# eth-cscs/COSTA

Measured on AMD Instinct MI355X. Metric: GB/s device-resident tile pack+transpose+unpack (fp64), % HBM peak, higher is better.
Workload: dtype f64; 1 GPU; pxtran fp64 16384x16384, 256x256 blocks, op T, alpha=1 beta=0, 1x1 grid (BASELINE configs[1]); op=T, parallelism=1 rank(s), one per GPU, RCCL send/recv exchange, m=16384, n=16384, block=256, grid=1x1

## Files before the change

costa_amd/__init__.py:

```python
from __future__ import annotations

import ctypes as C
import os
import struct
from dataclasses import dataclass
from typing import Iterable, Sequence

import numpy as np

__all__ = [
    "CostaError", "lib", "FLOAT", "DOUBLE", "CFLOAT", "CDOUBLE", "INT32", "dtype_code",
    "np_dtype", "Layout", "block_cyclic_layout", "custom_layout", "Comm", "transform",
    "transform_batch", "transform_async", "transform_batch_async", "synchronize", "transformer", "copy_and_transform", "execute_tiles", "execute_tiles_mixed",
    "convert_subtile", "TileOp",
    "plan_export", "set_profiling", "get_stats", "release_caches", "TILE_OP_DTYPE",
]

FLOAT, DOUBLE, CFLOAT, CDOUBLE, INT32 = 0, 1, 2, 3, 4
_NP = {FLOAT: np.float32, DOUBLE: np.float64, CFLOAT: np.complex64,
       CDOUBLE: np.complex128, INT32: np.int32}

TILE_TRANSPOSE, TILE_CONJ, TILE_VEC_SRC, TILE_VEC_DST = 0x1, 0x2, 0x4, 0x8
SCALE_BITCOPY, SCALE_ZERO, SCALE_ALPHA, SCALE_AXPBY = 0, 1, 2, 3

# ... 54 lines not shown
                ("plan_misses", C.c_int64), ("host_groups", C.c_int64),
                ("device_plans", C.c_int64), ("plan_ms", C.c_double), ("host_direct", C.c_int64),
                ("host_direct_groups", C.c_int64), ("tile_items", C.c_int64), ("skew_items", C.c_int64),
                ("cblock_items", C.c_int64), ("tiny_items", C.c_int64), ("device_lists", C.c_int64),
                ("fused_pieces", C.c_int64)]

    def as_dict(self) -> dict:
        out = {}
        for cls in reversed(type(self).__mro__):
            for k, _ in cls.__dict__.get("_fields_", ()):
                out[k] = getattr(self, k)
        return out


class FullStats(Stats):
    _fields_ = [("convert_items", C.c_int64)]


LIB_PATH = os.environ.get("COSTA_LIB") or os.path.join(os.path.dirname(os.path.abspath(__file__)),
                                                       "lib", "libcosta_amd.so")
_lib = None


def lib():
    global _lib
    if _lib is not None:
        return _lib
    if not os.environ.get("COSTA_NO_TORCH"):
        try:
            import torch
        except Exception:
# ... 2 lines not shown
        raise CostaError(-1, f"native library missing: {LIB_PATH} (run __graft_entry__.build())")
    L = C.CDLL(LIB_PATH, mode=C.RTLD_GLOBAL)
    vp, i, c, i64 = C.c_void_p, C.c_int, C.c_char, C.c_int64
    sig = {
        "costa_hip_last_error": (C.c_char_p, []),
        "costa_hip_version": (i, []),
        "costa_hip_block_cyclic_layout": (i, [i, i, i, i, i, i, i, i, i, i, i, c, i, i, vp, i, c, i,
                                              C.POINTER(vp)]),
        "costa_hip_custom_layout": (i, [i, i, i, C.POINTER(i), C.POINTER(i), C.POINTER(i), i,
                                        C.POINTER(_Block), c, C.POINTER(vp)]),
        "costa_hip_layout_destroy": (None, [vp]),
        "costa_hip_layout_reorder_ranks": (i, [vp, C.POINTER(i), i]),
        "costa_hip_layout_num_blocks": (i, [vp]),
        "costa_hip_layout_block": (i, [vp, i, C.POINTER(i), C.POINTER(i), C.POINTER(i),
                                       C.POINTER(i), C.POINTER(vp), C.POINTER(i)]),
        "costa_hip_comm_self": (i, [i, C.POINTER(vp)]),
        "costa_hip_comm_unique_id": (i, [C.c_char_p]),
        "costa_hip_comm_create": (i, [C.c_char_p, i, i, i, C.POINTER(vp)]),
        "costa_hip_comm_rank": (i, [vp]),
        "costa_hip_comm_size": (i, [vp]),
        "costa_hip_comm_destroy": (None, [vp]),
        "costa_hip_transform": (i, [vp, vp, c, vp, vp, vp]),
        "costa_hip_transform_batch": (i, [i, C.POINTER(vp), C.POINTER(vp), C.c_char_p, vp, vp,
                                          vp]),
        "costa_hip_transform_async": (i, [vp, vp, c, vp, vp, vp, vp]),
        "costa_hip_transform_batch_async": (i, [i, C.POINTER(vp), C.POINTER(vp), C.c_char_p, vp,
                                                vp, vp, vp]),
        "costa_hip_synchronize": (i, [vp]),
        "costa_hip_device_count": (i, [C.POINTER(i)]),
        "costa_hip_rccl_version": (i, [C.POINTER(i)]),
# ... 71 lines not shown

    @property
    def handle(self) -> C.c_void_p:
        return self._h

    def num_blocks(self) -> int:
        return lib().costa_hip_layout_num_blocks(self._h)

    def block(self, i: int) -> BlockInfo:
        v = [C.c_int() for _ in range(4)]
        d, ld = C.c_void_p(), C.c_int()
        _check(lib().costa_hip_layout_block(self._h, i, *[C.byref(x) for x in v], C.byref(d),
                                            C.byref(ld)))
        return BlockInfo(v[0].value, v[1].value, v[2].value, v[3].value, d.value or 0, ld.value)

    def reorder_ranks(self, reordering: Sequence[int]):
        p = np.ascontiguousarray(reordering, dtype=np.int32)
        _check(lib().costa_hip_layout_reorder_ranks(self._h, p.ctypes.data_as(C.POINTER(C.c_int)),
                                                    int(p.size)))

    def close(self):
        if self._h and self._h.value:
            lib().costa_hip_layout_destroy(self._h)
            self._h = C.c_void_p(0)

    def __del__(self):
        try:
            self.close()
        except Exception:
            pass
# ... 299 lines not shown
```

costa_amd/csrc/capi.cpp:

```cpp
#include "engine.hpp"

#include <hip/hip_runtime.h>

#include <costa/transform.hpp>

#include <algorithm>
#include <cctype>
#include <complex>
#include <cstring>
#include <new>

struct costa_layout_s {
    costa::engine::elayout e;
    std::vector<int> base_owners;
};
struct costa_comm_s {
    costa::engine::comm* c = nullptr;
};

namespace {
thread_local std::string g_last_error;

template <typename F>
int guarded(F&& f) {
// ... 201 lines not shown
            if (seen[size_t(reordering[k])]++)
                throw costa::engine::error(COSTA_ERR_ARG, "costa: reordering is not a permutation");
        }
        std::vector<int> owners(base.size());
        for (size_t k = 0; k < base.size(); ++k) owners[k] = n > 0 ? reordering[base[k]] : base[k];
        e.owners = std::move(owners);
        e.n_ranks = std::max(e.n_ranks, n);
        costa::engine::set_layout_hash(e);
    });
}

int costa_hip_layout_num_blocks(costa_layout_t layout) {
    return layout ? int(layout->e.blocks.size()) : -1;
}

int costa_hip_layout_block(costa_layout_t layout, int i, int* row_start, int* row_end,
                           int* col_start, int* col_end, void** data, int* ld) {
    return guarded([&] {
        if (!layout || i < 0 || size_t(i) >= layout->e.blocks.size())
            throw costa::engine::error(COSTA_ERR_ARG, "block index out of range");
        const auto& b = layout->e.blocks[size_t(i)];
        if (row_start) *row_start = b.rows.start;
        if (row_end) *row_end = b.rows.end;
        if (col_start) *col_start = b.cols.start;
        if (col_end) *col_end = b.cols.end;
        if (data) *data = b.data;
        if (ld) *ld = b.ld;
    });
}

// ... 319 lines not shown
```

costa_amd/csrc/convert_kernels.hip:

```cpp
#include <hip/hip_runtime.h>

#include <algorithm>
#include <string>
#include <type_traits>

#include "engine.hpp"
#include "tile_device.hpp"

#pragma clang fp contract(off)

namespace costa {
namespace engine {
namespace {

template <typename Td, typename Ts>
struct conv_t {
    static __device__ __forceinline__ Td of(Ts x) { return static_cast<Td>(x); }
};
template <typename Rd, typename Rs>
struct conv_t<cpx<Rd>, cpx<Rs>> {
    static __device__ __forceinline__ cpx<Rd> of(cpx<Rs> x) {
        return {static_cast<Rd>(x.re), static_cast<Rd>(x.im)};
    }
};
// ... 107 lines not shown
template <typename Ts, typename Td, bool FULL>
__device__ __forceinline__ void run_convert(const costa_tile_op_t& op, int f0, int s0, int tf_, int ts_,
                                            const char* src_base, char* dst_base, Td alpha, Td beta,
                                            typename cshape<Ts, Td>::Tn* tile) {
    using S = cshape<Ts, Td>;
    using Tn = typename S::Tn;
    constexpr int V = S::V, P = S::P;
    const int tf = FULL ? S::BF : tf_;
    const int ts = FULL ? S::BS : ts_;
    const uint32_t flags = op.flags;
    const uint32_t kind = (flags & COSTA_SCALE_MASK) >> COSTA_SCALE_SHIFT;
    const bool conj = flags & COSTA_TILE_CONJ;
    const bool vs = FULL || (flags & COSTA_TILE_VEC_SRC);
    const bool vd = FULL || (flags & COSTA_TILE_VEC_DST);
    const int64_t lds = op.lds, ldd = op.ldd;
    const Ts* src = reinterpret_cast<const Ts*>(src_base + op.src) + int64_t(s0) * lds + f0;

    const int lf = (int(threadIdx.x) % S::LPC) * V;
    const int c0 = int(threadIdx.x) / S::LPC;
    auto col_of = [&](int k) { return c0 + k * S::CPP; };
    const int nf_lane = FULL ? V : tf - lf;
    strip<Ts, V> x[S::PL];
#pragma unroll
    for (int k = 0; k < S::PL; ++k) {
        const int s = col_of(k);
        if (FULL || (nf_lane > 0 && s < ts)) sload(x[k], src + s * lds + lf, nf_lane, vs);
    }

    if (!(flags & COSTA_TILE_TRANSPOSE)) {
        Td* dst = reinterpret_cast<Td*>(dst_base + op.dst) + int64_t(s0) * ldd + f0;
        strip<Td, V> y[S::PL];
        if (kind == COSTA_SCALE_AXPBY) {
#pragma unroll
            for (int k = 0; k < S::PL; ++k) {
                const int s = col_of(k);
                if (FULL || (nf_lane > 0 && s < ts)) sload(y[k], dst + s * ldd + lf, nf_lane, vd);
            }
        }
        uint32_t redo = 0;
#pragma unroll
        for (int k = 0; k < S::PL; ++k) {
            const int s = col_of(k);
            if (!FULL && (nf_lane <= 0 || s >= ts)) continue;
            strip<Td, V> o;
            bool bad = false;
// ... 15 lines not shown
                    if (!((redo >> k) & 1u)) continue;
                    const int s = col_of(k);
                    const Ts* a = src + s * lds + lf;
                    Td* d = dst + s * ldd + lf;
                    const int n = FULL ? V : min(V, nf_lane);
#pragma unroll 1
                    for (int e = 0; e < n; ++e)
                        d[e] = scale(conv<Td>(a[e]), kind == COSTA_SCALE_AXPBY ? d[e] : e_zero<Td>(),
                                     kind, conj, alpha, beta);
                }
            }
        }
        return;
    }

    Td* dst = reinterpret_cast<Td*>(dst_base + op.dst) + int64_t(f0) * ldd + s0;
    const int lane = int(threadIdx.x) % 64, wave = int(threadIdx.x) / 64;
    constexpr int SW = S::SW, QG = S::QG;
    auto unit = [&](int k, int& f, int& sb, int& n) {
        const int u = wave + S::NW * k;
        const int sc = u / QG, q = u % QG;
        const int j = lane & (V - 1);
        f = q * V + j;
        sb = sc * SW + (lane - j);
        n = FULL ? V : ts - sb;
        return FULL || (f < tf && n > 0);
    };
    strip<Td, V> old[S::PS];
    if (kind == COSTA_SCALE_AXPBY) {
#pragma unroll
        for (int k = 0; k < S::PS; ++k) {
// ... 193 lines not shown
```

costa_amd/csrc/engine.cpp:

```cpp
#include <exception>
#include <thread>
#include "engine.hpp"

#include <hip/hip_runtime.h>
#include <rccl/rccl.h>

#include <algorithm>
#include <numeric>
#include <chrono>
#include <cmath>
#include <cstdio>
#include <cstdlib>
#include <cstring>
#include <deque>
#include <list>
#include <map>
#include <mutex>
#include <unordered_map>

namespace costa {
namespace engine {

#define HIP_CHECK(x)                                                                   \
    do {                                                                               \
// ... 1389 lines not shown
        h2 = (h2 + v) * 0x9fb21c651e98df25ull;
        h2 ^= h2 >> 31;
    }
    void mix_vec(const std::vector<int>& v) {
        mix(v.size());
        for (int x : v) mix(uint64_t(uint32_t(x)));
    }
    void mix_layout(const elayout& L) {
        mix(uint64_t(L.dtype));
        mix(uint64_t(uint8_t(L.ordering)));
        mix(uint64_t(L.n_ranks));
        mix_vec(L.rows_split);
        mix_vec(L.cols_split);
        mix_vec(L.owners);
        mix(L.blocks.size());
        for (const auto& b : L.blocks) {
            mix(uint64_t(uint32_t(b.rows.start)) | (uint64_t(uint32_t(b.rows.end)) << 32));
            mix(uint64_t(uint32_t(b.cols.start)) | (uint64_t(uint32_t(b.cols.end)) << 32));
            mix(reinterpret_cast<uintptr_t>(b.data));
            mix(uint64_t(uint32_t(b.ld)));
        }
    }
};

}

uint64_t layout_hash(const elayout& L) {
    hasher h;
    h.mix_layout(L);
    return h.h | 1;
}

void layout_hashes(const elayout& L, uint64_t& h1, uint64_t& h2) {
    hasher h;
    h.mix_layout(L);
    h1 = h.h | 1;
    h2 = h.h2;
}

// ... 8 lines not shown
    std::vector<hrange> h2d_ranges, d2h_ranges;
    dbuf stage;
    dbuf d_local, w_local, d_scal;
    work_split l_local;
    bool tr_local = true, ax_local = true;
    convert_list c_local;
    struct xround {
        dbuf d_pack, w_pack, d_unpack, w_unpack;
        work_split l_pack, l_unpack;
        convert_list c_pack, c_unpack;
        bool tr_unpack = false, ax_unpack = false;
    };
    std::vector<std::unique_ptr<xround>> rounds;
    std::vector<unsigned char> scal_host;
    std::shared_ptr<host_pipeline> pipe;
};

constexpr size_t kMaxPlans = 16;
struct keyed_plan {
    uint64_t h = 0;
    std::vector<uint64_t> key;
    std::unique_ptr<cached_plan> plan;
};
std::list<keyed_plan> g_plans;

void key_layout(std::vector<uint64_t>& k, const elayout& L) {
    uint64_t h1 = L.hash, h2 = L.hash2;
    if (!h1) layout_hashes(L, h1, h2);
    k.push_back(h1);
    k.push_back(h2);
    k.push_back(uint64_t(L.dtype) | uint64_t(uint8_t(L.ordering)) << 8 |
                uint64_t(uint32_t(L.n_ranks)) << 32);
    k.push_back(uint64_t(uint32_t(L.nbr())) | uint64_t(uint32_t(L.nbc())) << 32);
    k.push_back(L.blocks.size());
    if (!L.blocks.empty())
        for (const eblock* b : {&L.blocks.front(), &L.blocks.back()}) {
            k.push_back(reinterpret_cast<uintptr_t>(b->data));
            k.push_back(uint64_t(uint32_t(b->ld)) | uint64_t(uint32_t(b->rows.start)) << 32);
        }
// ... 139 lines not shown
        key_layout(key, *j.C);
        uint64_t w = uint64_t(uint8_t(std::toupper(static_cast<unsigned char>(j.trans))));
        for (bool cm : {true, false})
            w = w << 8 | scale_kind(j.C->dtype, j.s, cm, std::toupper(j.trans) == 'C');
        key.push_back(w);
    }
    hasher h;
    for (uint64_t w : key) h.mix(w);
    for (auto it = g_plans.begin(); it != g_plans.end(); ++it) {
        if (it->h == h.h && it->key == key) {
            g_plans.splice(g_plans.begin(), g_plans, it);
            g_stats.plan_hits++;
            return g_plans.front().plan.get();
        }
    }
    g_stats.plan_misses++;
    static const bool trace = std::getenv("COSTA_PLAN_TRACE") != nullptr;
    auto now = [] {
        return std::chrono::duration<double, std::milli>(
                   std::chrono::steady_clock::now().time_since_epoch()).count();
    };
    const double t0 = now();
    double t_resid = 0, t_plan = 0, t_work = 0;

    const bool mixed = any_mixed(jobs);
    if (mixed) {
        costa_dtype_t a, b;
        check_jobs(jobs, c->size, a, b);
    }
    auto cp = std::make_unique<cached_plan>();
    cp->device = c->device;
    bool all_dev = true;
    std::vector<const elayout*> host_layouts;
    std::vector<bool> on_dev;
    for (const auto& j : jobs)
        for (const elayout* L : {j.A, j.C}) {
            bool d = layout_on_device(*L);
            on_dev.push_back(d);
            all_dev = all_dev && d;
        }
    std::vector<elayout> remapped;
    std::vector<job> pj = jobs;
    std::vector<hrange> staged_ranges;
    std::vector<uint8_t> range_flags;
    if (!all_dev && mixed)
        throw error(COSTA_ERR_ARG,
                    "costa: mixed-precision transforms (A and C of different element types) need "
                    "device-resident layouts");
    if (!all_dev) {
        cp->staged = true;
        std::vector<const elayout*> As, Cs;
        size_t k = 0;
        for (const auto& j : jobs) {
            if (!on_dev[k++]) As.push_back(j.A);
            if (!on_dev[k++]) Cs.push_back(j.C);
// ... 37 lines not shown
                       std::none_of(on_dev.begin(), on_dev.end(), [](bool d) { return d; });
        for (uint8_t f : range_flags)
            if ((f & 3) == 3 || (f & 4)) pipe_ok = false;
        if (pipe_ok) {
            const double tp = now();
            auto hplan = plan_jobs(jobs, c, dc.main);
            g_stats.plan_ms += now() - tp;
            if (host_pipeline_accepts(hplan->dtype, hplan->pack_ops)) {
                cp->staged = false;
                cp->p = std::move(hplan);
                const int R = c->nccl ? exchange_rounds() : 1;
                std::vector<int> pr, ur;
                exchange_round_of_ops(*cp->p, R, pr, ur);
                cp->pipe = make_host_pipeline(cp->p->dtype, cp->p->pack_ops, cp->p->local_ops,
                                              cp->p->unpack_ops, pr, ur, R);
                g_plans.push_front({h.h, std::move(key), std::move(cp)});
                while (g_plans.size() > kMaxPlans) g_plans.pop_back();
                return g_plans.front().plan.get();
            }
        }
        cp->stage.reserve(std::max<size_t>(off, 256));
        staged_ranges = ranges;
        remapped.reserve(jobs.size() * 2);
        k = 0;
        for (auto& j : pj) {
            if (!on_dev[k++]) {
                remapped.push_back(remap(*j.A, ranges, static_cast<char*>(cp->stage.p)));
                j.A = &remapped.back();
            }
            if (!on_dev[k++]) {
                remapped.push_back(remap(*j.C, ranges, static_cast<char*>(cp->stage.p)));
// ... 88 lines not shown
        auto& x = *cp->rounds[size_t(r)];
        const device_section& su = sec_u[size_t(r)];
        x.d_pack.upload(ord_p[size_t(r)], dc.main);
        x.w_pack.upload(w_p[size_t(r)], dc.main);
        upload_list(x.d_unpack, ord_u[size_t(r)], su.d_ordered, su.at_ordered, su.n_ordered, dc.main);
        upload_list(x.w_unpack, w_u[size_t(r)], su.d_work, su.at_work, su.n_work, dc.main);
    }
    HIP_CHECK(hipStreamSynchronize(dc.main));
    if (trace)
        std::fprintf(stderr,
                     "[costa plan] %zu local / %zu pack / %zu unpack ops: residency %.2f ms, "
                     "planning %.2f, work lists %.2f, upload %.2f, total %.2f\n",
                     p.local_ops.size(), p.pack_ops.size(), p.unpack_ops.size(), t_resid, t_plan,
                     t_work, now() - t0 - t_resid - t_plan - t_work, now() - t0);

    g_plans.push_front({h.h, std::move(key), std::move(cp)});
    while (g_plans.size() > kMaxPlans) g_plans.pop_back();
    return g_plans.front().plan.get();
}

void upload_scalars(cached_plan& cp, const std::vector<job>& jobs, hipStream_t s) {
    const size_t E = dtype_size(cp.p->dtype);
    std::vector<unsigned char> host(jobs.size() * 2 * E);
    for (size_t t = 0; t < jobs.size(); ++t) {
        std::memcpy(&host[(2 * t) * E], jobs[t].s.alpha.data(), E);
        std::memcpy(&host[(2 * t + 1) * E], jobs[t].s.beta.data(), E);
    }
    if (host != cp.scal_host || !cp.d_scal.p) {
        cp.d_scal.reserve(host.size());
        cp.scal_host = host;
        HIP_CHECK(hipMemcpyAsync(cp.d_scal.p, cp.scal_host.data(), host.size(),
// ... 151 lines not shown
            HIP_CHECK(hipMemcpyAsync(static_cast<char*>(cp.stage.p) + r.dev_off,
                                     reinterpret_cast<void*>(r.lo), r.hi - r.lo,
                                     hipMemcpyHostToDevice, dc.main));
        tm.stop();
    }

    const bool exchange = c->nccl != nullptr && (p.send_elems > 0 || p.recv_elems > 0);
    hipStream_t ls = exchange ? dc.aux : dc.main;
    if (exchange) {
        HIP_CHECK(hipEventRecord(dc.ev_ready, dc.main));
        HIP_CHECK(hipStreamWaitEvent(dc.aux, dc.ev_ready, 0));
    }
    if (cp.c_local.n_items) {
        tm.start(PH_LOCAL, ls);
        launch_convert(p.src_dtype, p.dtype, static_cast<const costa_tile_op_t*>(cp.d_local.p),
                       static_cast<const uint64_t*>(cp.w_local.p), cp.c_local, nullptr, nullptr,
                       cp.d_scal.p, ls);
        tm.stop();
    }
    if (cp.l_local.n_items()) {
        tm.start(PH_LOCAL, ls);
        launch_tiles(p.dtype,
                     make_launch(cp.l_local, cp.d_local.p, cp.w_local.p, nullptr, nullptr,
                                 cp.d_scal.p, cp.tr_local, cp.ax_local),
                     ls);
        tm.stop();
    }

    if (exchange) {
        dc.send.reserve(size_t(p.send_elems) * E + 256);
        dc.recv.reserve(size_t(p.recv_elems) * E + 256);
        char* sb = static_cast<char*>(dc.send.p);
        char* rb = static_cast<char*>(dc.recv.p);
        const int R = int(cp.rounds.size());
        dc.round_events(size_t(R));
        for (int r = 0; r < R; ++r) {
            const auto& x = *cp.rounds[size_t(r)];
            if (x.c_pack.n_items) {
                tm.start(PH_PACK, dc.main);
                launch_convert(p.src_dtype, p.pkg_dtype, static_cast<const costa_tile_op_t*>(x.d_pack.p),
                               static_cast<const uint64_t*>(x.w_pack.p), x.c_pack, nullptr, sb,
                               cp.d_scal.p, dc.main);
                tm.stop();
            }
            if (x.l_pack.n_items()) {
                tm.start(PH_PACK, dc.main);
                launch_tiles(p.pkg_dtype,
                             make_launch(x.l_pack, x.d_pack.p, x.w_pack.p, nullptr, sb, cp.d_scal.p,
                                         false, false),
                             dc.main);
                tm.stop();
            }
            HIP_CHECK(hipEventRecord(dc.ev_packed[size_t(r)], dc.main));
            HIP_CHECK(hipStreamWaitEvent(dc.xch, dc.ev_packed[size_t(r)], 0));
            tm.start(PH_EXCHANGE, dc.xch);
            issue_exchange(c, p, sb, rb, dc.xch, r, R);
            tm.stop();
            HIP_CHECK(hipEventRecord(dc.ev_moved[size_t(r)], dc.xch));
        }
        for (int r = 0; r < R; ++r) {
            const auto& x = *cp.rounds[size_t(r)];
            if (x.c_unpack.n_items) {
                HIP_CHECK(hipStreamWaitEvent(dc.aux, dc.ev_moved[size_t(r)], 0));
                tm.start(PH_UNPACK, dc.aux);
                launch_convert(p.pkg_dtype, p.dtype, static_cast<const costa_tile_op_t*>(x.d_unpack.p),
                               static_cast<const uint64_t*>(x.w_unpack.p), x.c_unpack, rb, nullptr,
                               cp.d_scal.p, dc.aux);
                tm.stop();
            }
            if (!x.l_unpack.n_items()) continue;
            HIP_CHECK(hipStreamWaitEvent(dc.aux, dc.ev_moved[size_t(r)], 0));
            tm.start(PH_UNPACK, dc.aux);
            launch_tiles(p.dtype,
                         make_launch(x.l_unpack, x.d_unpack.p, x.w_unpack.p, rb, nullptr,
                                     cp.d_scal.p, x.tr_unpack, x.ax_unpack),
                         dc.aux);
            tm.stop();
        }
        HIP_CHECK(hipEventRecord(dc.ev_local, dc.aux));
        HIP_CHECK(hipStreamWaitEvent(dc.main, dc.ev_local, 0));
        HIP_CHECK(hipStreamWaitEvent(dc.main, dc.ev_moved[size_t(R - 1)], 0));
    }

    if (cp.staged) {
        tm.start(PH_D2H, dc.main);
        for (const auto& r : cp.d2h_ranges)
            HIP_CHECK(hipMemcpyAsync(reinterpret_cast<void*>(r.lo),
                                     static_cast<char*>(cp.stage.p) + r.dev_off, r.hi - r.lo,
                                     hipMemcpyDeviceToHost, dc.main));
// ... 126 lines not shown
```

costa_amd/csrc/engine.hpp:

```cpp
#pragma once

#include <costa/layout.hpp>
#include <costa_hip.h>

#include <array>
#include <cstdint>
#include <functional>
#include <memory>
#include <string>
#include <vector>

namespace costa {
namespace engine {

size_t dtype_size(costa_dtype_t t);
bool dtype_is_complex(costa_dtype_t t);

struct eblock {
    interval rows, cols;
    char* data = nullptr;
    int ld = 0;
};

struct elayout {
    costa_dtype_t dtype = COSTA_DOUBLE;
    std::vector<int> rows_split, cols_split;
    std::vector<int> owners;
    int n_ranks = 1;
    char ordering = 'C';
    std::vector<eblock> blocks;
    uint64_t hash = 0;
    uint64_t hash2 = 0;

    int nbr() const { return int(rows_split.size()) - 1; }
    int nbc() const { return int(cols_split.size()) - 1; }
};

template <typename T>
costa_dtype_t dtype_of();

template <typename T>
elayout erase(const grid_layout<T>& L);

uint64_t layout_hash(const elayout& L);
void layout_hashes(const elayout& L, uint64_t& h1, uint64_t& h2);
void set_layout_hash(elayout& L);

struct scal {
    std::array<unsigned char, 16> alpha{};
    std::array<unsigned char, 16> beta{};
};

struct job {
    const elayout* A = nullptr;
    const elayout* C = nullptr;
    char trans = 'N';
    scal s;
};
// ... 217 lines not shown
```

costa_amd/csrc/tile_device.hpp:

```cpp
#pragma once

#include <hip/hip_runtime.h>

#include <cstdint>

#include "costa_hip.h"

#pragma clang fp contract(off)

namespace costa {
namespace engine {
namespace {

template <typename R>
struct cpx {
    R re, im;
};

template <typename T> __device__ __forceinline__ T e_mul(T a, T b) { return a * b; }
template <typename T> __device__ __forceinline__ T e_add(T a, T b) { return a + b; }
template <typename T> __device__ __forceinline__ T e_conj(T a) { return a; }
template <typename T> __device__ __forceinline__ T e_zero() { return T(0); }

template <typename R>
__device__ __attribute__((cold)) cpx<R> annex_g_recover(R a, R b, R c, R d) {
    const R one = R(1), zero = R(0), inf = __builtin_huge_val();
    const bool ovf = __builtin_isinf(a * c) || __builtin_isinf(b * d) || __builtin_isinf(a * d) ||
                     __builtin_isinf(b * c);
    bool recalc = false;
    if (__builtin_isinf(a) || __builtin_isinf(b)) {
        a = __builtin_copysign(__builtin_isinf(a) ? one : zero, a);
        b = __builtin_copysign(__builtin_isinf(b) ? one : zero, b);
// ... 218 lines not shown
```

costa_amd/csrc/tile_kernels.hip:

```cpp
#include <hip/hip_runtime.h>

#include <algorithm>
#include <cstdlib>
#include <type_traits>

#include "engine.hpp"
#include "tile_device.hpp"

#pragma clang fp contract(off)

namespace costa {
namespace engine {
namespace {

template <typename T, int V, int EPS>
__device__ __forceinline__ vec<T> shifted_chunk(const vec<T>& below, const vec<T>& o) {
    vec<T> c;
#pragma unroll
    for (int e = 0; e < V; ++e)
        c.e[e] = e < EPS ? below.e[V - EPS + e < V ? V - EPS + e : V - 1] : o.e[e >= EPS ? e - EPS : 0];
    return c;
}
template <typename T, typename S, bool NT>
__device__ __forceinline__ void store_shifted(T* d, const vec<T>& o, int n, int lane) {
// ... 115 lines not shown
typedef const __attribute__((address_space(1))) void glob_void;

template <typename T, typename S, bool FULL, bool NT = true>
__device__ __forceinline__ void run_tile(const costa_tile_op_t& op, int f0, int s0, int tf_, int ts_,
                                         const char* src_base, char* dst_base, T alpha, T beta,
                                         T* tile) {
    constexpr int V = S::V, BF = S::BF, P = S::P;
    const int tf = FULL ? S::BF : tf_;
    const int ts = FULL ? S::BS : ts_;
    const uint32_t flags = op.flags;
    const uint32_t kind = (flags & COSTA_SCALE_MASK) >> COSTA_SCALE_SHIFT;
    const bool conj = flags & COSTA_TILE_CONJ;
    const bool vs = FULL || (flags & COSTA_TILE_VEC_SRC);
    const bool vd = FULL || (flags & COSTA_TILE_VEC_DST);
    const int64_t lds = op.lds, ldd = op.ldd;
    const T* src = reinterpret_cast<const T*>(src_base + op.src) + int64_t(s0) * lds + f0;

    const int lf = (int(threadIdx.x) % S::LPC) * V;
    const int c0 = int(threadIdx.x) / S::LPC;
    auto col_of = [&](int k) { return c0 + k * S::CPP; };
    const int nf_lane = FULL ? V : tf - lf;
    vec<T> x[S::PL];
#pragma unroll
    for (int k = 0; k < S::PL; ++k) {
        const int s = col_of(k);
        if (FULL || (nf_lane > 0 && s < ts)) vload(x[k], src + s * lds + lf, nf_lane, vs);
    }

    if (!(flags & COSTA_TILE_TRANSPOSE)) {
        T* dst = reinterpret_cast<T*>(dst_base + op.dst) + int64_t(s0) * ldd + f0;
        vec<T> y[S::PL];
        if (kind == COSTA_SCALE_AXPBY) {
#pragma unroll
            for (int k = 0; k < S::PL; ++k) {
                const int s = col_of(k);
                if (FULL || (nf_lane > 0 && s < ts)) vload(y[k], dst + s * ldd + lf, nf_lane, vd);
            }
        }
        uint32_t redo = 0;
#pragma unroll
        for (int k = 0; k < S::PL; ++k) {
            const int s = col_of(k);
            if (!FULL && (nf_lane <= 0 || s >= ts)) continue;
            T* d = dst + s * ldd + lf;
            if (kind != COSTA_SCALE_BITCOPY) {
// ... 17 lines not shown
                    if (!((redo >> k) & 1u)) continue;
                    const int s = col_of(k);
                    const T* a = src + s * lds + lf;
                    T* d = dst + s * ldd + lf;
                    const int n = FULL ? V : min(V, nf_lane);
#pragma unroll 1
                    for (int e = 0; e < n; ++e)
                        d[e] = scale(a[e], kind == COSTA_SCALE_AXPBY ? d[e] : e_zero<T>(), kind, conj,
                                     alpha, beta);
                }
            }
        }
        return;
    }

    T* dst = reinterpret_cast<T*>(dst_base + op.dst) + int64_t(f0) * ldd + s0;
    const int lane = int(threadIdx.x) % 64, wave = int(threadIdx.x) / 64;
    constexpr int SW = S::SW, FW = S::FW, QG = BF / V / FW;
    constexpr int NSC = S::BS / SW;
    constexpr bool PAIR = FULL && std::is_same<T, double>::value && S::BF == 64 && S::BS == 128 && S::NT == 512;
    auto unit_u = [&](int k) {
        if constexpr (PAIR) return wave * S::PS + k;
        return wave + S::NW * k;
    };
    auto unit_sc = [&](int u) {
        if constexpr (PAIR) return u % NSC;
        return u / QG;
    };
    auto unit_q = [&](int u) {
        if constexpr (PAIR) return u / NSC;
        return u % QG;
// ... 131 lines not shown
    extern __shared__ __attribute__((aligned(16))) unsigned char smem[];
    T* tile = reinterpret_cast<T*>(smem);
    const uint64_t w = work[blockIdx.x];
    const costa_tile_op_t op = ops[w >> 32];
    const uint32_t sub = uint32_t(w);
    const int nbf = (op.nf + BF - 1) / BF;
    const int f0 = int(sub % uint32_t(nbf)) * BF;
    const int s0 = int(sub / uint32_t(nbf)) * BS;
    const int tf = min(BF, op.nf - f0), ns = op.ns;
    const uint32_t kind = (op.flags & COSTA_SCALE_MASK) >> COSTA_SCALE_SHIFT;
    const uint32_t slot = op.flags >> COSTA_SLOT_SHIFT;
    const T alpha = kind >= COSTA_SCALE_ALPHA ? scalars[2 * slot] : T(0);
    const T beta = kind == COSTA_SCALE_AXPBY ? scalars[2 * slot + 1] : T(0);
    const bool vs = op.flags & COSTA_TILE_VEC_SRC;
    const int64_t lds = op.lds, ldd = op.ldd;
    const T* src = reinterpret_cast<const T*>(src_base + op.src) + f0;
    const int lf = (int(threadIdx.x) % K::LPC) * V;
    const int c0 = int(threadIdx.x) / K::LPC;
    const int nf_lane = tf - lf;
    const int s_lo = s0 > 0 ? s0 - G : 0, s_hi = min(ns, s0 + BS);
    vec<T> x[K::PL];
#pragma unroll
    for (int k = 0; k < K::PL; ++k) {
        const int r = c0 + k * K::CPP, s = s0 - G + r;
        if (r < K::RS && s >= s_lo && s < s_hi && nf_lane > 0)
            vload<T, false>(x[k], src + s * lds + lf, nf_lane, vs);
    }
#pragma unroll
    for (int k = 0; k < K::PL; ++k) {
        const int r = c0 + k * K::CPP, s = s0 - G + r;
        if (r < K::RS && s >= s_lo && s < s_hi && nf_lane > 0) {
#pragma unroll
            for (int e = 0; e < V; ++e)
                if (e < nf_lane) tile[r * P + lf + e] = x[k].e[e];
        }
    }
    __syncthreads();
    const int lane = int(threadIdx.x) % 64, wave = int(threadIdx.x) / 64;
    T* dst = reinterpret_cast<T*>(dst_base + op.dst);
    const bool last = s0 + BS >= ns;
    for (int f = wave; f < tf; f += K::NW) {
        T* col = dst + int64_t(f0 + f) * ldd;
        const int eps = int((reinterpret_cast<uintptr_t>(col + s0) / sizeof(T)) & uintptr_t(G - 1));
        const int lo = s0 > 0 ? s0 - eps : 0;
        const int hi = last ? ns : s0 + BS - eps;
        const int mis = int((reinterpret_cast<uintptr_t>(col + lo) / sizeof(T)) & uintptr_t(V - 1));
        const int a = min(hi, lo + ((V - mis) & (V - 1)));
        const int b = a + (hi - a) / V * V;
        const T* tcol = tile + (G - s0) * P + f;
        if (lo + lane < a) {
            T* d = col + lo + lane;
            *d = scale(tcol[(lo + lane) * P], kind == COSTA_SCALE_AXPBY ? *d : T(0), kind, false, alpha, beta);
        }
        if (b + lane < hi) {
// ... 121 lines not shown
}

template <typename T, bool TR, bool AX, int UC>
__device__ __forceinline__ void tiny_op(const costa_tile_op_t& op, int lane, T* t,
                                        const char* src_base, char* dst_base,
                                        const T* __restrict__ scalars) {
    const uint32_t flags = op.flags;
    const uint32_t kind = (flags & COSTA_SCALE_MASK) >> COSTA_SCALE_SHIFT;
    const bool conj = flags & COSTA_TILE_CONJ;
    const uint32_t slot = flags >> COSTA_SLOT_SHIFT;
    T alpha = e_zero<T>(), beta = e_zero<T>();
    if (kind >= COSTA_SCALE_ALPHA) {
        alpha = scalars[2 * slot];
        beta = scalars[2 * slot + 1];
    }
    const T* src = reinterpret_cast<const T*>(src_base + op.src);
    T* dst = reinterpret_cast<T*>(dst_base + op.dst);
    const int nf = op.nf, ns = op.ns, total = nf * ns;
    const int64_t lds = op.lds, ldd = op.ldd;

    if (!TR || !(flags & COSTA_TILE_TRANSPOSE)) {
        constexpr int UCE = UC / int(sizeof(T)) > 0 ? UC / int(sizeof(T)) : 1;
        lin<T> p(lane, nf);
        for (int e0 = 0; e0 < total; e0 += 64 * UCE) {
            T x[UCE];
            T y[AX ? UCE : 1];
            const lin<T> q0 = p;
#pragma unroll
            for (int u = 0; u < UCE; ++u) {
                if (e0 + u * 64 >= total) break;
                if (e0 + u * 64 + lane < total) x[u] = src[p.s * lds + p.f];
                p.step();
// ... 58 lines not shown
    const uint64_t h = work[g];
    const costa_tile_op_t hd = ops[h];
    const int n_ops = int(hd.src), R = hd.nf, K = hd.ns, P = R | 1;
    const uint32_t flags = hd.flags;
    const uint32_t kind = (flags & COSTA_SCALE_MASK) >> COSTA_SCALE_SHIFT;
    const bool conj = flags & COSTA_TILE_CONJ;
    const bool tr = TR && (flags & COSTA_TILE_TRANSPOSE);
    const uint32_t slot = flags >> COSTA_SLOT_SHIFT;
    T alpha = e_zero<T>(), beta = e_zero<T>();
    if (kind >= COSTA_SCALE_ALPHA) {
        alpha = scalars[2 * slot];
        beta = scalars[2 * slot + 1];
    }
    const int lane = int(threadIdx.x) % 64;
    const int wave = __builtin_amdgcn_readfirstlane(int(threadIdx.x) / 64);
    T* dst = reinterpret_cast<T*>(dst_base + hd.dst);
    const int total = R * K;
    const int mis = int((reinterpret_cast<uintptr_t>(dst) / sizeof(T)) & uintptr_t(V - 1));
    const int nvec = (total + mis + V - 1) / V;
    vec<T> old[CB_CHUNKS];
    if (AX && kind == COSTA_SCALE_AXPBY) {
#pragma unroll
        for (int k = 0; k < CB_CHUNKS; ++k) {
            const int c = int(threadIdx.x) + CB_NT * k;
            const int e0 = V * c - mis;
            if (c >= nvec) break;
            if (e0 >= 0 && e0 + V <= total) {
                raw16 r = *reinterpret_cast<const raw16*>(dst + e0);
                __builtin_memcpy(&old[k], &r, 16);
            } else {
#pragma unroll
                for (int e = 0; e < V; ++e)
                    if (e0 + e >= 0 && e0 + e < total) old[k].e[e] = dst[e0 + e];
            }
        }
    }
    for (int i = wave; i < n_ops; i += NW) {
        const costa_tile_op_t op = ops[h + 1 + uint64_t(i)];
        const T* src = reinterpret_cast<const T*>(src_base + op.src);
        const int64_t e0 = int64_t(op.dst - hd.dst) / int64_t(sizeof(T));
        const int r0 = int(e0 % R), c0 = int(e0 / R);
        const int nf = op.nf, n = op.nf * op.ns;
        const int64_t lds = op.lds;
        const int di_f = tr ? P : 1, di_s = tr ? 1 : P;
        const int ibase = c0 * P + r0;
        if constexpr (sizeof(T) == 4 && !TR) {
            const int ncm = (nf + 6) / 4, nq = ncm * op.ns;
            lin<T> q(lane, ncm);
            for (int b = 0; b < nq; b += 64 * CB_UV) {
                raw16 x[CB_UV];
                int fb[CB_UV], sv[CB_UV];
#pragma unroll
                for (int u = 0; u < CB_UV; ++u) {
                    fb[u] = nf;
// ... 296 lines not shown
```

include/costa_hip.h:

```cpp
#ifndef COSTA_HIP_H
#define COSTA_HIP_H

#include <stddef.h>
#include <stdint.h>

#ifdef __cplusplus
extern "C" {
#endif

#define COSTA_OK 0
#define COSTA_ERR_ARG 1
#define COSTA_ERR_HIP 2
#define COSTA_ERR_NCCL 3
#define COSTA_ERR_INTERNAL 4

typedef enum {
    COSTA_FLOAT = 0,
    COSTA_DOUBLE = 1,
    COSTA_CFLOAT = 2,
    COSTA_CDOUBLE = 3,
    COSTA_INT32 = 4
} costa_dtype_t;

typedef struct costa_layout_s* costa_layout_t;
// ... 34 lines not shown
int costa_hip_device_count(int* count);
int costa_hip_rccl_version(int* version);

int costa_hip_block_cyclic_layout(costa_dtype_t dtype, int m, int n, int block_m, int block_n,
                                  int i, int j, int sub_m, int sub_n, int p_m, int p_n,
                                  char rank_grid_ordering, int rsrc, int csrc, void* ptr, int lld,
                                  char data_ordering, int rank, costa_layout_t* out);
int costa_hip_custom_layout(costa_dtype_t dtype, int rowblocks, int colblocks, const int* rowsplit,
                            const int* colsplit, const int* owners, int nlocalblocks,
                            const costa_block_t* localblocks, char ordering, costa_layout_t* out);
void costa_hip_layout_destroy(costa_layout_t layout);
int costa_hip_layout_reorder_ranks(costa_layout_t layout, const int* reordering, int n);
int costa_hip_layout_num_blocks(costa_layout_t layout);
int costa_hip_layout_block(costa_layout_t layout, int i, int* row_start, int* row_end,
                           int* col_start, int* col_end, void** data, int* ld);

int costa_hip_comm_self(int device, costa_comm_t* out);
int costa_hip_comm_unique_id(unsigned char id[128]);
int costa_hip_comm_create(const unsigned char id[128], int nranks, int rank, int device,
                          costa_comm_t* out);
int costa_hip_comm_rank(costa_comm_t comm);
int costa_hip_comm_size(costa_comm_t comm);
void costa_hip_comm_destroy(costa_comm_t comm);

int costa_hip_transform(costa_layout_t A, costa_layout_t C, char trans, const void* alpha,
                        const void* beta, costa_comm_t comm);
int costa_hip_transform_batch(int n, const costa_layout_t* A, const costa_layout_t* C,
                              const char* trans, const void* alpha, const void* beta,
                              costa_comm_t comm);

// ... 37 lines not shown
typedef struct {
    double pack_ms, local_ms, unpack_ms, exchange_ms, h2d_ms, d2h_ms;
    int64_t pack_launches, local_launches, unpack_launches;
    int64_t pack_bytes, local_bytes, unpack_bytes;
    int64_t transforms;
    int64_t plan_hits, plan_misses;
    int64_t host_groups;
    int64_t device_plans;
    double plan_ms;
    int64_t host_direct;
    int64_t host_direct_groups;
    int64_t tile_items, skew_items, cblock_items, tiny_items;
    int64_t device_lists;
    int64_t fused_pieces;
    int64_t convert_items;
} costa_stats_t;
int costa_hip_set_profiling(int on);
int costa_hip_get_stats(costa_stats_t* out, int reset);
int costa_hip_release_caches(void);

int costa_hip_set_host_staging(int mode);

int costa_hip_set_planner(int mode);
int costa_hip_plan_export_device(int device, int n, const costa_layout_t* A, const costa_layout_t* C,
                                 const char* trans, const void* alpha, const void* beta, int rank,
                                 int nranks, costa_plan_info_t* info, costa_tile_op_t* local_ops,
                                 costa_tile_op_t* pack_ops, costa_tile_op_t* unpack_ops,
                                 int64_t* send_counts, int64_t* send_displs, int64_t* recv_counts,
                                 int64_t* recv_displs, void* scalars);

// ... 10 lines not shown
```

Baseline: 6217 GB/s.

## Rebind cached device plans to shifted buffer addresses instead of replanning

Adds a relative plan key that ignores absolute buffer base addresses for device-resident layouts, so a cached plan can be reused when the same layout shape shows up at a different allocation. The reused plan gets a base delta, which the pack, local and unpack kernels add to their offsets. It also caches the on-device residency check per layout and makes the kernels form pointers in the global address space. This removes replanning and plan upload when callers pass freshly allocated buffers, at the cost of extra key building and an offset add on every pointer in the kernels.

```diff
diff --git a/costa_amd/__init__.py b/costa_amd/__init__.py
--- a/costa_amd/__init__.py
+++ b/costa_amd/__init__.py
@@ -92,7 +92,8 @@
 
 
 class FullStats(Stats):
-    _fields_ = [("convert_items", C.c_int64)]
+    _fields_ = [("convert_items", C.c_int64), ("plan_rebinds", C.c_int64),
+                ("rebind_ms", C.c_double)]
 
 
 LIB_PATH = os.environ.get("COSTA_LIB") or os.path.join(os.path.dirname(os.path.abspath(__file__)),
@@ -125,6 +126,7 @@
         "costa_hip_layout_num_blocks": (i, [vp]),
         "costa_hip_layout_block": (i, [vp, i, C.POINTER(i), C.POINTER(i), C.POINTER(i),
                                        C.POINTER(i), C.POINTER(vp), C.POINTER(i)]),
+        "costa_hip_layout_key": (i, [vp, C.POINTER(C.c_uint64)]),
         "costa_hip_comm_self": (i, [i, C.POINTER(vp)]),
         "costa_hip_comm_unique_id": (i, [C.c_char_p]),
         "costa_hip_comm_create": (i, [C.c_char_p, i, i, i, C.POINTER(vp)]),
@@ -226,6 +228,11 @@
                                             C.byref(ld)))
         return BlockInfo(v[0].value, v[1].value, v[2].value, v[3].value, d.value or 0, ld.value)
 
+    def key(self) -> tuple:
+        k = (C.c_uint64 * 4)()
+        _check(lib().costa_hip_layout_key(self._h, k))
+        return tuple(int(x) for x in k)
+
     def reorder_ranks(self, reordering: Sequence[int]):
         p = np.ascontiguousarray(reordering, dtype=np.int32)
         _check(lib().costa_hip_layout_reorder_ranks(self._h, p.ctypes.data_as(C.POINTER(C.c_int)),
diff --git a/costa_amd/csrc/capi.cpp b/costa_amd/csrc/capi.cpp
--- a/costa_amd/csrc/capi.cpp
+++ b/costa_amd/csrc/capi.cpp
@@ -239,6 +239,17 @@
     return layout ? int(layout->e.blocks.size()) : -1;
 }
 
+int costa_hip_layout_key(costa_layout_t layout, uint64_t key[4]) {
+    return guarded([&] {
+        if (!layout || !key) throw costa::engine::error(COSTA_ERR_ARG, "null argument");
+        const uint64_t base = costa::engine::layout_base(layout->e);
+        key[0] = layout->e.hash;
+        key[1] = layout->e.hash2;
+        key[2] = base % costa::engine::kRebindQuantum;
+        key[3] = base;
+    });
+}
+
 int costa_hip_layout_block(costa_layout_t layout, int i, int* row_start, int* row_end,
                            int* col_start, int* col_end, void** data, int* ld) {
     return guarded([&] {
diff --git a/costa_amd/csrc/convert_kernels.hip b/costa_amd/csrc/convert_kernels.hip
--- a/costa_amd/csrc/convert_kernels.hip
+++ b/costa_amd/csrc/convert_kernels.hip
@@ -145,7 +145,7 @@
     const bool vs = FULL || (flags & COSTA_TILE_VEC_SRC);
     const bool vd = FULL || (flags & COSTA_TILE_VEC_DST);
     const int64_t lds = op.lds, ldd = op.ldd;
-    const Ts* src = reinterpret_cast<const Ts*>(src_base + op.src) + int64_t(s0) * lds + f0;
+    const Ts* src = list_ptr<const Ts>(src_base, op.src) + int64_t(s0) * lds + f0;
 
     const int lf = (int(threadIdx.x) % S::LPC) * V;
     const int c0 = int(threadIdx.x) / S::LPC;
@@ -159,7 +159,7 @@
     }
 
     if (!(flags & COSTA_TILE_TRANSPOSE)) {
-        Td* dst = reinterpret_cast<Td*>(dst_base + op.dst) + int64_t(s0) * ldd + f0;
+        Td* dst = list_ptr<Td>(dst_base, op.dst) + int64_t(s0) * ldd + f0;
         strip<Td, V> y[S::PL];
         if (kind == COSTA_SCALE_AXPBY) {
 #pragma unroll
@@ -205,7 +205,7 @@
         return;
     }
 
-    Td* dst = reinterpret_cast<Td*>(dst_base + op.dst) + int64_t(f0) * ldd + s0;
+    Td* dst = list_ptr<Td>(dst_base, op.dst) + int64_t(f0) * ldd + s0;
     const int lane = int(threadIdx.x) % 64, wave = int(threadIdx.x) / 64;
     constexpr int SW = S::SW, QG = S::QG;
     auto unit = [&](int k, int& f, int& sb, int& n) {
diff --git a/costa_amd/csrc/engine.cpp b/costa_amd/csrc/engine.cpp
--- a/costa_amd/csrc/engine.cpp
+++ b/costa_amd/csrc/engine.cpp
@@ -1427,15 +1427,20 @@
         mix_vec(L.cols_split);
         mix_vec(L.owners);
         mix(L.blocks.size());
+        const uint64_t base = layout_base(L);
         for (const auto& b : L.blocks) {
             mix(uint64_t(uint32_t(b.rows.start)) | (uint64_t(uint32_t(b.rows.end)) << 32));
             mix(uint64_t(uint32_t(b.cols.start)) | (uint64_t(uint32_t(b.cols.end)) << 32));
-            mix(reinterpret_cast<uintptr_t>(b.data));
+            mix(uint64_t(reinterpret_cast<uintptr_t>(b.data)) - base);
             mix(uint64_t(uint32_t(b.ld)));
         }
     }
 };
 
+}
+
+uint64_t layout_base(const elayout& L) {
+    return L.blocks.empty() ? 0 : uint64_t(reinterpret_cast<uintptr_t>(L.blocks.front().data));
 }
 
 uint64_t layout_hash(const elayout& L) {
@@ -1474,6 +1479,10 @@
     std::vector<std::unique_ptr<xround>> rounds;
     std::vector<unsigned char> scal_host;
     std::shared_ptr<host_pipeline> pipe;
+    uint64_t a0 = 0, c0 = 0;
+    uint64_t dA = 0, dC = 0;
+    const char* src_shift() const { return reinterpret_cast<const char*>(uintptr_t(dA)); }
+    char* dst_shift() const { return reinterpret_cast<char*>(uintptr_t(dC)); }
 };
 
 constexpr size_t kMaxPlans = 16;
@@ -1481,8 +1490,43 @@
     uint64_t h = 0;
     std::vector<uint64_t> key;
     std::unique_ptr<cached_plan> plan;
+    uint64_t rh = 0;
+    std::vector<uint64_t> rkey;
 };
 std::list<keyed_plan> g_plans;
+
+uint64_t batch_anchor(const std::vector<job>& jobs, bool c_side) {
+    for (const job& j : jobs) {
+        const elayout& L = c_side ? *j.C : *j.A;
+        if (!L.blocks.empty()) return layout_base(L);
+    }
+    return 0;
+}
+
+bool resident(const elayout& L) {
+    if (L.hash && L.on_device >= 0) return L.on_device != 0;
+    const bool d = layout_on_device(L);
+    if (L.hash) L.on_device = d ? 1 : 0;
+    return d;
+}
+
+void rel_key_layout(std::vector<uint64_t>& k, const elayout& L, uint64_t h1, uint64_t h2, bool on_dev,
+                    uint64_t anchor) {
+    k.push_back(h1);
+    k.push_back(h2);
+    k.push_back(uint64_t(L.dtype) | uint64_t(uint8_t(L.ordering)) << 8 | uint64_t(on_dev) << 16 |
+                uint64_t(uint32_t(L.n_ranks)) << 32);
+    k.push_back(uint64_t(uint32_t(L.nbr())) | uint64_t(uint32_t(L.nbc())) << 32);
+    k.push_back(L.blocks.size());
+    if (L.blocks.empty()) return;
+    const uint64_t base = layout_base(L);
+    k.push_back(base % kRebindQuantum);
+    k.push_back(base - anchor);
+    for (const eblock* b : {&L.blocks.front(), &L.blocks.back()})
+        k.push_back(uint64_t(uint32_t(b->ld)) | uint64_t(uint32_t(b->rows.start)) << 32);
+}
+
+size_t key_layout_words(const elayout& L) { return L.blocks.empty() ? 5 : 9; }
 
 void key_layout(std::vector<uint64_t>& k, const elayout& L) {
     uint64_t h1 = L.hash, h2 = L.hash2;
@@ -1652,13 +1696,49 @@
             return g_plans.front().plan.get();
         }
     }
-    g_stats.plan_misses++;
-    static const bool trace = std::getenv("COSTA_PLAN_TRACE") != nullptr;
     auto now = [] {
         return std::chrono::duration<double, std::milli>(
                    std::chrono::steady_clock::now().time_since_epoch()).count();
     };
     const double t0 = now();
+    bool all_dev = true;
+    std::vector<bool> on_dev;
+    for (const auto& j : jobs)
+        for (const elayout* L : {j.A, j.C}) {
+            const bool d = resident(*L);
+            on_dev.push_back(d);
+            all_dev = all_dev && d;
+        }
+    const uint64_t anchor_a = batch_anchor(jobs, false), anchor_c = batch_anchor(jobs, true);
+    std::vector<uint64_t> rkey;
+    hasher rh;
+    if (all_dev) {
+        rkey.reserve(3 + jobs.size() * 20);
+        rkey.insert(rkey.end(), key.begin(), key.begin() + 3);
+        size_t at = 3;
+        for (const auto& j : jobs) {
+            rel_key_layout(rkey, *j.A, key[at], key[at + 1], true, anchor_a);
+            at += key_layout_words(*j.A);
+            rel_key_layout(rkey, *j.C, key[at], key[at + 1], true, anchor_c);
+            at += key_layout_words(*j.C);
+            rkey.push_back(key[at++]);
+        }
+        for (uint64_t w : rkey) rh.mix(w);
+        for (auto it = g_plans.begin(); it != g_plans.end(); ++it) {
+            if (it->rkey.empty() || it->rh != rh.h || it->rkey != rkey) continue;
+            it->h = h.h;
+            it->key = std::move(key);
+            it->plan->dA = anchor_a - it->plan->a0;
+            it->plan->dC = anchor_c - it->plan->c0;
+            g_plans.splice(g_plans.begin(), g_plans, it);
+            g_stats.plan_hits++;
+            g_stats.plan_rebinds++;
+            g_stats.rebind_ms += now() - t0;
+            return g_plans.front().plan.get();
+        }
+    }
+    g_stats.plan_misses++;
+    static const bool trace = std::getenv("COSTA_PLAN_TRACE") != nullptr;
     double t_resid = 0, t_plan = 0, t_work = 0;
 
     const bool mixed = any_mixed(jobs);
@@ -1668,15 +1748,8 @@
     }
     auto cp = std::make_unique<cached_plan>();
     cp->device = c->device;
-    bool all_dev = true;
-    std::vector<const elayout*> host_layouts;
-    std::vector<bool> on_dev;
-    for (const auto& j : jobs)
-        for (const elayout* L : {j.A, j.C}) {
-            bool d = layout_on_device(*L);
-            on_dev.push_back(d);
-            all_dev = all_dev && d;
-        }
+    cp->a0 = anchor_a;
+    cp->c0 = anchor_c;
     std::vector<elayout> remapped;
     std::vector<job> pj = jobs;
     std::vector<hrange> staged_ranges;
@@ -1744,7 +1817,7 @@
                 exchange_round_of_ops(*cp->p, R, pr, ur);
                 cp->pipe = make_host_pipeline(cp->p->dtype, cp->p->pack_ops, cp->p->local_ops,
                                               cp->p->unpack_ops, pr, ur, R);
-                g_plans.push_front({h.h, std::move(key), std::move(cp)});
+                g_plans.push_front({h.h, std::move(key), std::move(cp), 0, {}});
                 while (g_plans.size() > kMaxPlans) g_plans.pop_back();
                 return g_plans.front().plan.get();
             }
@@ -1863,7 +1936,7 @@
                      p.local_ops.size(), p.pack_ops.size(), p.unpack_ops.size(), t_resid, t_plan,
                      t_work, now() - t0 - t_resid - t_plan - t_work, now() - t0);
 
-    g_plans.push_front({h.h, std::move(key), std::move(cp)});
+    g_plans.push_front({h.h, std::move(key), std::move(cp), rh.h, std::move(rkey)});
     while (g_plans.size() > kMaxPlans) g_plans.pop_back();
     return g_plans.front().plan.get();
 }
@@ -2045,15 +2118,15 @@
     if (cp.c_local.n_items) {
         tm.start(PH_LOCAL, ls);
         launch_convert(p.src_dtype, p.dtype, static_cast<const costa_tile_op_t*>(cp.d_local.p),
-                       static_cast<const uint64_t*>(cp.w_local.p), cp.c_local, nullptr, nullptr,
-                       cp.d_scal.p, ls);
+                       static_cast<const uint64_t*>(cp.w_local.p), cp.c_local, cp.src_shift(),
+                       cp.dst_shift(), cp.d_scal.p, ls);
         tm.stop();
     }
     if (cp.l_local.n_items()) {
         tm.start(PH_LOCAL, ls);
         launch_tiles(p.dtype,
-                     make_launch(cp.l_local, cp.d_local.p, cp.w_local.p, nullptr, nullptr,
-                                 cp.d_scal.p, cp.tr_local, cp.ax_local),
+                     make_launch(cp.l_local, cp.d_local.p, cp.w_local.p, cp.src_shift(),
+                                 cp.dst_shift(), cp.d_scal.p, cp.tr_local, cp.ax_local),
                      ls);
         tm.stop();
     }
@@ -2070,15 +2143,15 @@
             if (x.c_pack.n_items) {
                 tm.start(PH_PACK, dc.main);
                 launch_convert(p.src_dtype, p.pkg_dtype, static_cast<const costa_tile_op_t*>(x.d_pack.p),
-                               static_cast<const uint64_t*>(x.w_pack.p), x.c_pack, nullptr, sb,
+                               static_cast<const uint64_t*>(x.w_pack.p), x.c_pack, cp.src_shift(), sb,
                                cp.d_scal.p, dc.main);
                 tm.stop();
             }
             if (x.l_pack.n_items()) {
                 tm.start(PH_PACK, dc.main);
                 launch_tiles(p.pkg_dtype,
-                             make_launch(x.l_pack, x.d_pack.p, x.w_pack.p, nullptr, sb, cp.d_scal.p,
-                                         false, false),
+                             make_launch(x.l_pack, x.d_pack.p, x.w_pack.p, cp.src_shift(), sb,
+                                         cp.d_scal.p, false, false),
                              dc.main);
                 tm.stop();
             }
@@ -2095,7 +2168,7 @@
                 HIP_CHECK(hipStreamWaitEvent(dc.aux, dc.ev_moved[size_t(r)], 0));
                 tm.start(PH_UNPACK, dc.aux);
                 launch_convert(p.pkg_dtype, p.dtype, static_cast<const costa_tile_op_t*>(x.d_unpack.p),
-                               static_cast<const uint64_t*>(x.w_unpack.p), x.c_unpack, rb, nullptr,
+                               static_cast<const uint64_t*>(x.w_unpack.p), x.c_unpack, rb, cp.dst_shift(),
                                cp.d_scal.p, dc.aux);
                 tm.stop();
             }
@@ -2103,7 +2176,7 @@
             HIP_CHECK(hipStreamWaitEvent(dc.aux, dc.ev_moved[size_t(r)], 0));
             tm.start(PH_UNPACK, dc.aux);
             launch_tiles(p.dtype,
-                         make_launch(x.l_unpack, x.d_unpack.p, x.w_unpack.p, rb, nullptr,
+                         make_launch(x.l_unpack, x.d_unpack.p, x.w_unpack.p, rb, cp.dst_shift(),
                                      cp.d_scal.p, x.tr_unpack, x.ax_unpack),
                          dc.aux);
             tm.stop();
diff --git a/costa_amd/csrc/engine.hpp b/costa_amd/csrc/engine.hpp
--- a/costa_amd/csrc/engine.hpp
+++ b/costa_amd/csrc/engine.hpp
@@ -31,6 +31,7 @@
     std::vector<eblock> blocks;
     uint64_t hash = 0;
     uint64_t hash2 = 0;
+    mutable int on_device = -1;
 
     int nbr() const { return int(rows_split.size()) - 1; }
     int nbc() const { return int(cols_split.size()) - 1; }
@@ -42,6 +43,8 @@
 template <typename T>
 elayout erase(const grid_layout<T>& L);
 
+uint64_t layout_base(const elayout& L);
+constexpr uint64_t kRebindQuantum = 256;
 uint64_t layout_hash(const elayout& L);
 void layout_hashes(const elayout& L, uint64_t& h1, uint64_t& h2);
 void set_layout_hash(elayout& L);
diff --git a/costa_amd/csrc/tile_device.hpp b/costa_amd/csrc/tile_device.hpp
--- a/costa_amd/csrc/tile_device.hpp
+++ b/costa_amd/csrc/tile_device.hpp
@@ -16,6 +16,12 @@
 struct cpx {
     R re, im;
 };
+
+template <typename T>
+__device__ __forceinline__ T* list_ptr(const char* base, uint64_t off) {
+    typedef T __attribute__((address_space(1))) * global_ptr;
+    return (T*)(global_ptr)(reinterpret_cast<uint64_t>(base) + off);
+}
 
 template <typename T> __device__ __forceinline__ T e_mul(T a, T b) { return a * b; }
 template <typename T> __device__ __forceinline__ T e_add(T a, T b) { return a + b; }
diff --git a/costa_amd/csrc/tile_kernels.hip b/costa_amd/csrc/tile_kernels.hip
--- a/costa_amd/csrc/tile_kernels.hip
+++ b/costa_amd/csrc/tile_kernels.hip
@@ -153,7 +153,7 @@
     const bool vs = FULL || (flags & COSTA_TILE_VEC_SRC);
     const bool vd = FULL || (flags & COSTA_TILE_VEC_DST);
     const int64_t lds = op.lds, ldd = op.ldd;
-    const T* src = reinterpret_cast<const T*>(src_base + op.src) + int64_t(s0) * lds + f0;
+    const T* src = list_ptr<const T>(src_base, op.src) + int64_t(s0) * lds + f0;
 
     const int lf = (int(threadIdx.x) % S::LPC) * V;
     const int c0 = int(threadIdx.x) / S::LPC;
@@ -167,7 +167,7 @@
     }
 
     if (!(flags & COSTA_TILE_TRANSPOSE)) {
-        T* dst = reinterpret_cast<T*>(dst_base + op.dst) + int64_t(s0) * ldd + f0;
+        T* dst = list_ptr<T>(dst_base, op.dst) + int64_t(s0) * ldd + f0;
         vec<T> y[S::PL];
         if (kind == COSTA_SCALE_AXPBY) {
 #pragma unroll
@@ -215,7 +215,7 @@
         return;
     }
 
-    T* dst = reinterpret_cast<T*>(dst_base + op.dst) + int64_t(f0) * ldd + s0;
+    T* dst = list_ptr<T>(dst_base, op.dst) + int64_t(f0) * ldd + s0;
     const int lane = int(threadIdx.x) % 64, wave = int(threadIdx.x) / 64;
     constexpr int SW = S::SW, FW = S::FW, QG = BF / V / FW;
     constexpr int NSC = S::BS / SW;
@@ -377,7 +377,7 @@
     const T beta = kind == COSTA_SCALE_AXPBY ? scalars[2 * slot + 1] : T(0);
     const bool vs = op.flags & COSTA_TILE_VEC_SRC;
     const int64_t lds = op.lds, ldd = op.ldd;
-    const T* src = reinterpret_cast<const T*>(src_base + op.src) + f0;
+    const T* src = list_ptr<const T>(src_base, op.src) + f0;
     const int lf = (int(threadIdx.x) % K::LPC) * V;
     const int c0 = int(threadIdx.x) / K::LPC;
     const int nf_lane = tf - lf;
@@ -400,7 +400,7 @@
     }
     __syncthreads();
     const int lane = int(threadIdx.x) % 64, wave = int(threadIdx.x) / 64;
-    T* dst = reinterpret_cast<T*>(dst_base + op.dst);
+    T* dst = list_ptr<T>(dst_base, op.dst);
     const bool last = s0 + BS >= ns;
     for (int f = wave; f < tf; f += K::NW) {
         T* col = dst + int64_t(f0 + f) * ldd;
@@ -552,8 +552,8 @@
         alpha = scalars[2 * slot];
         beta = scalars[2 * slot + 1];
     }
-    const T* src = reinterpret_cast<const T*>(src_base + op.src);
-    T* dst = reinterpret_cast<T*>(dst_base + op.dst);
+    const T* src = list_ptr<const T>(src_base, op.src);
+    T* dst = list_ptr<T>(dst_base, op.dst);
     const int nf = op.nf, ns = op.ns, total = nf * ns;
     const int64_t lds = op.lds, ldd = op.ldd;
 
@@ -642,7 +642,7 @@
     }
     const int lane = int(threadIdx.x) % 64;
     const int wave = __builtin_amdgcn_readfirstlane(int(threadIdx.x) / 64);
-    T* dst = reinterpret_cast<T*>(dst_base + hd.dst);
+    T* dst = list_ptr<T>(dst_base, hd.dst);
     const int total = R * K;
     const int mis = int((reinterpret_cast<uintptr_t>(dst) / sizeof(T)) & uintptr_t(V - 1));
     const int nvec = (total + mis + V - 1) / V;
@@ -665,7 +665,7 @@
     }
     for (int i = wave; i < n_ops; i += NW) {
         const costa_tile_op_t op = ops[h + 1 + uint64_t(i)];
-        const T* src = reinterpret_cast<const T*>(src_base + op.src);
+        const T* src = list_ptr<const T>(src_base, op.src);
         const int64_t e0 = int64_t(op.dst - hd.dst) / int64_t(sizeof(T));
         const int r0 = int(e0 % R), c0 = int(e0 / R);
         const int nf = op.nf, n = op.nf * op.ns;
diff --git a/include/costa_hip.h b/include/costa_hip.h
--- a/include/costa_hip.h
+++ b/include/costa_hip.h
@@ -72,6 +72,7 @@
 int costa_hip_layout_num_blocks(costa_layout_t layout);
 int costa_hip_layout_block(costa_layout_t layout, int i, int* row_start, int* row_end,
                            int* col_start, int* col_end, void** data, int* ld);
+int costa_hip_layout_key(costa_layout_t layout, uint64_t key[4]);
 
 int costa_hip_comm_self(int device, costa_comm_t* out);
 int costa_hip_comm_unique_id(unsigned char id[128]);
@@ -139,6 +140,8 @@
     int64_t device_lists;
     int64_t fused_pieces;
     int64_t convert_items;
+    int64_t plan_rebinds;
+    double rebind_ms;
 } costa_stats_t;
 int costa_hip_set_profiling(int on);
 int costa_hip_get_stats(costa_stats_t* out, int reset);
```

Result: no change. 6218 GB/s (median of 5 runs) (+0.0%).
